# fegemo/palette-and-histo-gan

Measured on AMD Instinct MI355X. Metric: train images/sec (64x64x4 sprites), higher is better.
Workload: dtype bf16

## Files before the change

### include/p2pgan.h

```cpp
#ifndef P2PGAN_H
#define P2PGAN_H

#ifdef __cplusplus
extern "C" {
#endif

typedef enum { P2P_F32 = 0, P2P_BF16 = 1 } p2p_dtype;
typedef enum { P2P_OP_G = 0, P2P_OP_P = 1, P2P_OP_W = 2 } p2p_convop;
typedef enum { P2P_ACT_NONE = 0, P2P_ACT_LEAKY = 1, P2P_ACT_RELU = 2 } p2p_act;

typedef struct {
    void* ptr;
    long long img_stride;
    int row_stride;
    int ld;
} p2p_tensor;

typedef struct {
    const void* ptr;
    int kind;
    int nslabs;
    long long slab_stride;
    int ld;
    int coff;
} p2p_gsrc;

const char* p2p_last_error(void);
int p2p_version(void);
int p2p_view_halo_pixels(void);


int p2p_conv_direct(int op, int stride, int dtype, int N, int LH, int LW, int Cg, int Cd,
                    const p2p_tensor* hi, const p2p_tensor* lo, const void* w, const float* bias,
                    float* dw, float* dbias, void* stream);

int p2p_igemm(int op, int dtype, int N, int LH, int LW, int Cg, int Cd,
              const p2p_tensor* hi, const p2p_tensor* lo, const void* w,
              int splitk, float* slabs, float* stat_part, void* stream);
int p2p_igemm_stat_slots(int op, int N, int LH, int LW, int ncols);

int p2p_brig_ok(int op, int dtype, int N, int LH, int LW, int Cg, int Cd);
int p2p_igemm_norm_act_ok(int op, int dtype, int N, int LH, int LW, int Cg, int Cd);
int p2p_igemm_norm_act(int op, int dtype, int N, int LH, int LW, int Cg, int Cd, const p2p_tensor* hi, const p2p_tensor* lo,
                       const void* w, const float* gamma, const float* beta, float eps, int act, float alpha,
                       const p2p_tensor* act_out, float* stats, void* stream);
int p2p_brig_stat_slots(int op, int dtype, int N, int LH, int LW, int Cg, int Cd);
int p2p_igemm_layer_stat_slots(int op, int dtype, int N, int LH, int LW, int Cg, int Cd);

int p2p_igemm_edge(int op, int stride, int dtype, int N, int LH, int LW, int cin_pad, int ncols, int w_rows,
                   const p2p_tensor* in, const p2p_tensor* out, const void* w, const float* bias,
                   int act, float alpha, void* stream);

int p2p_conv_strip_ok(int op, int dtype, int N, int LH, int LW, int Cg, int Cd);
int p2p_conv_strip_stat_slots(int op, int dtype, int N, int LH, int LW, int Cg, int Cd);
int p2p_conv_strip(int op, int dtype, int N, int LH, int LW, int Cg, int Cd,
                   const p2p_tensor* hi, const p2p_tensor* lo, const void* w, float* stat_part, void* stream);

int p2p_conv_fewout_ok(int op, int stride, int dtype, int N, int LH, int LW, int cin_pad, int ncols);
int p2p_conv_fewout(int op, int stride, int dtype, int N, int LH, int LW, int cin_pad, int ncols, int w_rows,
                    const p2p_tensor* in, const p2p_tensor* out, const void* w, const float* bias,
                    int act, float alpha, void* stream);

int p2p_conv_fewin_ok(int op, int stride, int dtype, int N, int LH, int LW, int cin_pad, int ncols);
int p2p_conv_fewin(int op, int stride, int dtype, int N, int LH, int LW, int cin_pad, int ncols, int w_rows,
                   const p2p_tensor* in, const p2p_tensor* out, const void* w, const float* bias,
                   int act, float alpha, void* stream);

int p2p_conv_fewin_actbwd(int op, int stride, int dtype, int N, int LH, int LW, int cin_pad, int ncols, int w_rows,
                          const p2p_tensor* in, const p2p_tensor* out, const void* w, const p2p_tensor* gate, float alpha,
                          void* stream);

long long p2p_wgemm_workspace_bytes(int N, int LH, int LW, int Cg, int Cd, int msplit);
int p2p_wgemm(int dtype, int N, int LH, int LW, int Cg, int Cd,
              const p2p_tensor* hi, const p2p_tensor* lo, float* dw,
              int msplit, void* workspace, void* stream);

int p2p_wgemm_edge(int dtype, int stride, int N, int LH, int LW, int Cg, int Cd,
                   const p2p_tensor* hi, const p2p_tensor* lo, float* dw,
                   int msplit, void* workspace, void* stream);

int p2p_wgrad_small_blocks(int dtype, int stride, int N, int LH, int LW, int Cg, int Cd, int hi_ld, int lo_ld);
int p2p_wgrad_small(int dtype, int stride, int N, int LH, int LW, int Cg, int Cd,
                    const p2p_tensor* hi, const p2p_tensor* lo, float* dw, void* workspace, void* stream);

long long p2p_view_colsum_workspace_bytes(int dtype, int N, int H, int W, int C, const p2p_tensor* v);
int p2p_view_colsum(int dtype, int N, int H, int W, int C, const p2p_tensor* v, float* out, float* workspace, void* stream);



#define P2P_IGEMM_FAM_R03 1
#define P2P_IGEMM_FAM_GEN 2
#define P2P_IGEMM_FAM_PIPE_G 3
#define P2P_IGEMM_FAM_PIPE_P 4
#define P2P_IGEMM_TILE_128x128 0
#define P2P_IGEMM_TILE_256x128 1
#define P2P_IGEMM_TILE_128x64 2
#define P2P_IGEMM_TILE_256x64 3
#define P2P_IGEMM_TILE_128x32 4
#define P2P_IGEMM_TILE_256x32 5
#define P2P_IGEMM_ROUTE(family, tile, kgroups, stages, w_major) \
    ((family) | ((tile) << 3) | (((kgroups) - 1) << 6) | (((stages) - 2) << 7) | ((w_major) << 9))
#define P2P_IGEMM_ROUTE_BRIG 0
#define P2P_IGEMM_ARMS(X) \
    X(1, 0, 1, 2) X(1, 0, 1, 3) X(1, 1, 1, 2) X(1, 1, 1, 3) X(1, 2, 1, 2) X(1, 2, 1, 3) \
    X(1, 3, 1, 2) X(1, 3, 1, 3) X(1, 4, 1, 2) X(1, 4, 1, 3) X(1, 5, 1, 2) X(1, 5, 1, 3) \
    X(2, 0, 1, 2) X(2, 0, 1, 3) X(2, 1, 1, 2) X(2, 1, 1, 3) X(2, 2, 1, 2) X(2, 2, 1, 3) \
    X(2, 3, 1, 2) X(2, 3, 1, 3) X(2, 4, 1, 2) X(2, 4, 1, 3) X(2, 5, 1, 2) X(2, 5, 1, 3) \
    X(3, 1, 1, 3) X(3, 0, 2, 4) X(3, 0, 1, 2) X(4, 1, 1, 3) X(4, 0, 2, 4) X(4, 0, 1, 2)
int p2p_igemm_route(int op, int dtype, int N, int LH, int LW, int Cg, int Cd, const p2p_tensor* hi, const p2p_tensor* lo,
                    int splitk, int with_stats);
int p2p_igemm_edge_route(int op, int stride, int dtype, int N, int LH, int LW, int cin_pad, int ncols, int w_rows,
                         const p2p_tensor* in, const p2p_tensor* out, int with_bias, int act);

#define P2P_BRIG_ROUTE(op_p, cbw, stagger, fused) (1 | ((op_p) << 1) | (((cbw) - 1) << 2) | ((stagger) << 3) | ((fused) << 4))
#define P2P_BRIG_ROUTE_NONE 0
#define P2P_BRIG_ARMS(X) \
    X(0, 1, 0, 0) X(0, 1, 0, 1) X(0, 1, 1, 0) X(0, 1, 1, 1) X(0, 2, 0, 0) X(0, 2, 0, 1) X(0, 2, 1, 0) X(0, 2, 1, 1) \
    X(1, 1, 0, 0) X(1, 1, 0, 1) X(1, 1, 1, 0) X(1, 1, 1, 1) X(1, 2, 0, 0) X(1, 2, 0, 1) X(1, 2, 1, 0) X(1, 2, 1, 1)
int p2p_brig_route(int op, int dtype, int N, int LH, int LW, int Cg, int Cd, int fused);

#define P2P_WGEMM_ROUTE_PIPE 0
#define P2P_WGEMM_ROUTE_128x128 1
#define P2P_WGEMM_ROUTE_64x128 2
#define P2P_WGEMM_ROUTE_32x128 3
#define P2P_WGEMM_ROUTE_64x64 4
#define P2P_WGEMM_ROUTE_32x64 5
#define P2P_WGEMM_ROUTE_64x32 6
#define P2P_WGEMM_ROUTE_32x32 7
#define P2P_WGEMM_ARMS(X) X(0) X(1) X(2) X(3) X(4) X(5) X(6) X(7)
int p2p_wgemm_route(int dtype, int stride, int N, int LH, int LW, int Cg, int Cd, const p2p_tensor* hi, const p2p_tensor* lo,
                    int msplit);

#define P2P_WS_TILE_1x1 0
#define P2P_WS_TILE_1x2 1
#define P2P_WS_TILE_1x4 2
#define P2P_WS_TILE_2x1 3
#define P2P_WS_TILE_2x2 4
#define P2P_WS_ROUTE(stride, tile, waves, pack, swizzle) \
    (((stride) - 1) | ((tile) << 1) | (((waves) >> 4) << 4) | ((pack) << 5) | ((swizzle) << 7))
#define P2P_WS_ARMS(X) \
    X(1, 0, 8, 0, 0) X(1, 0, 8, 0, 1) X(1, 0, 16, 0, 0) X(1, 0, 16, 0, 1) X(1, 1, 8, 0, 0) X(1, 1, 8, 0, 1) X(1, 1, 16, 0, 0) X(1, 1, 16, 0, 1) \
    X(1, 2, 8, 0, 0) X(1, 2, 8, 0, 1) X(1, 2, 16, 0, 0) X(1, 2, 16, 0, 1) X(1, 3, 8, 0, 0) X(1, 3, 8, 0, 1) X(1, 3, 16, 0, 0) X(1, 3, 16, 0, 1) \
    X(1, 4, 8, 0, 0) X(1, 4, 8, 0, 1) X(1, 4, 16, 0, 0) X(1, 4, 16, 0, 1) \
    X(2, 0, 8, 0, 0) X(2, 0, 8, 0, 1) X(2, 0, 16, 0, 0) X(2, 0, 16, 0, 1) X(2, 1, 8, 0, 0) X(2, 1, 8, 0, 1) X(2, 1, 16, 0, 0) X(2, 1, 16, 0, 1) \
    X(2, 2, 8, 0, 0) X(2, 2, 8, 0, 1) X(2, 2, 16, 0, 0) X(2, 2, 16, 0, 1) X(2, 3, 8, 0, 0) X(2, 3, 8, 0, 1) X(2, 3, 16, 0, 0) X(2, 3, 16, 0, 1) \
    X(2, 4, 8, 0, 0) X(2, 4, 8, 0, 1) X(2, 4, 16, 0, 0) X(2, 4, 16, 0, 1) \
    X(1, 1, 8, 1, 0) X(2, 1, 8, 1, 0) X(1, 3, 8, 2, 0)
int p2p_wgrad_small_route(int dtype, int stride, int N, int LH, int LW, int Cg, int Cd, int hi_ld, int lo_ld);

#define P2P_NORM_FORM_SCALAR 0
#define P2P_NORM_FORM_SMALL 1
#define P2P_NORM_FORM_REG 2
#define P2P_NORM_FORM_VEC0 3
#define P2P_NORM_FORM_VEC12 4
#define P2P_NORM_FORM_VEC3 5
#define P2P_NORM_ROUTE(form, ppl, slabs, lg_cg) ((form) | ((ppl) << 3) | ((slabs) << 7) | ((lg_cg) << 8))
#define P2P_NORM_ROUTE_ARM(code) ((code) & 0xff)
#define P2P_NORM_FWD_ARMS(X) \
    X(0, 0, 0) X(1, 1, 0) X(1, 1, 1) X(1, 2, 0) X(1, 2, 1) X(1, 4, 0) X(1, 4, 1) \
    X(2, 1, 0) X(2, 1, 1) X(2, 2, 0) X(2, 2, 1) X(2, 4, 0) X(2, 4, 1) X(2, 8, 0) X(2, 8, 1) X(3, 0, 0) X(4, 0, 0) X(5, 0, 0)
#define P2P_NORM_BWD_ARMS(X) \
    X(0, 0, 0) X(1, 1, 0) X(1, 1, 1) X(1, 2, 0) X(1, 2, 1) X(1, 4, 0) X(1, 4, 1) \
    X(2, 1, 0) X(2, 1, 1) X(2, 2, 0) X(2, 2, 1) X(2, 4, 0) X(2, 4, 1) X(2, 8, 0) X(2, 8, 1) X(3, 0, 0) X(4, 0, 0)
int p2p_norm_act_fwd_route(int dtype, int N, int H, int W, int C, const void* raw, int raw_kind, int nslabs,
                           long long slab_stride, const float* gamma, const float* beta, const p2p_tensor* out,
                           void* raw_out, float* stats, float* ws, long long ws_bytes, int nsplit,
                           const p2p_tensor* tail, int tail_ch);
int p2p_norm_act_bwd_route(int dtype, int N, int H, int W, int C, const void* raw, const float* stats, const float* gamma,
                           const float* beta, const p2p_gsrc* g1, const p2p_gsrc* g2, const p2p_tensor* draw,
                           float* dgamma_part, float* dbeta_part, float* ws, long long ws_bytes, int nsplit);


int p2p_norm_act_fwd(int dtype, int N, int H, int W, int C,
                     const void* raw, int raw_kind, int nslabs, long long slab_stride,
                     const float* gamma, const float* beta, float eps, int act, float alpha,
                     const unsigned char* mask, const p2p_tensor* out, void* raw_out, float* stats,
                     float* ws, long long ws_bytes, int nsplit, void* stream);
int p2p_norm_act_fwd_tail(int dtype, int N, int H, int W, int C,
                          const void* raw, int raw_kind, int nslabs, long long slab_stride,
                          const float* gamma, const float* beta, float eps, int act, float alpha,
                          const unsigned char* mask, const p2p_tensor* out, void* raw_out, float* stats,
                          float* ws, long long ws_bytes, int nsplit, const p2p_tensor* tail, int tail_ch, void* stream);

int p2p_norm_act_bwd(int dtype, int N, int H, int W, int C,
                     const void* raw, const float* stats, const float* gamma, const float* beta,
                     int act, float alpha, const unsigned char* mask,
                     const p2p_gsrc* g1, const p2p_gsrc* g2,
                     const p2p_tensor* draw, float* dgamma_part, float* dbeta_part,
                     float* ws, long long ws_bytes, int nsplit, void* stream);

int p2p_norm_act_fwd_1x1(int dtype, int N, int C, const float* gamma, const float* beta, int act, float alpha,
                         const unsigned char* mask, const p2p_tensor* out, void* stream);
int p2p_norm_act_bwd_1x1(int dtype, int N, int C, const float* gamma, const float* beta, int act, float alpha,
                         const unsigned char* mask, const p2p_gsrc* g1, const p2p_gsrc* g2, float* dgamma_part,
                         float* dbeta_part, void* stream);

int p2p_act_bwd(int dtype, int N, int H, int W, int C, const p2p_tensor* act_out, const p2p_gsrc* g1,
                const p2p_gsrc* g2, float alpha, const p2p_tensor* draw, void* stream);

int p2p_colsum(const float* part, int rows, int cols, float scale, float* out, void* stream);

int p2p_colsum_batched(const float* part, const int* table, int ntasks, int max_cols, float* out, void* stream);


#define P2P_LOSS_BLOCKS 256
int p2p_loss_partials_sum(const float* partials, int K, float* out, void* stream);

int p2p_bce_logits(int dtype, int N2, int n_real, int H, int W, const p2p_tensor* logits,
                   float inv_count, const p2p_tensor* dlogits_d, const p2p_tensor* dlogits_g,
                   float* partials, void* stream);
int p2p_bce_logits_pad8(int dtype, int N2, int n_real, int H, int W, const p2p_tensor* logits,
                        float inv_count, const p2p_tensor* dlogits_d, const p2p_tensor* dlogits_g,
                        float* partials, void* stream);

int p2p_tanh_l1_fwd(int dtype, int N, int H, int W, int C, const p2p_tensor* z, const p2p_tensor* real,
                    const p2p_tensor* fake, float inv_count, float* partials, float* fake_f32, void* stream);
int p2p_tanh_l1_fwd_pair(int dtype, int N, int H, int W, const p2p_tensor* z, const p2p_tensor* real_pair,
                         const p2p_tensor* fake_pair, float inv_count, float* partials, float* fake_f32, void* stream);

int p2p_tanh_l1_bwd(int dtype, int N, int H, int W, int C, const p2p_tensor* fake, const p2p_tensor* real,
                    const p2p_gsrc* g_d, const p2p_gsrc* g_extra, float l1_scale,
                    const p2p_tensor* dz, void* stream);
int p2p_tanh_l1_bwd_pad8(int dtype, int N, int H, int W, const p2p_tensor* fake, const p2p_tensor* real,
                         const p2p_gsrc* g_d, const p2p_gsrc* g_extra, float l1_scale, const p2p_tensor* dz,
                         void* stream);


int p2p_rgbuv_hist_fwd(int dtype, int N, int H, int W, const p2p_tensor* img, float* hist, void* stream);
int p2p_rgbuv_hist_general(int dtype, int N, int H, int W, const p2p_tensor* img, int size, int method, float sigma, float* hist,
                           void* stream);

long long p2p_rgbuv_hist_fwd3_workspace_bytes(int N);
int p2p_rgbuv_hist_fwd3(int dtype, int N, int H, int W, const p2p_tensor* img, const float* points, const int* npoints, int cap,
                        float* hist, float* workspace, void* stream);
int p2p_rgbuv_points(int dtype, int N, int H, int W, const p2p_tensor* img, int cap, float* points, int* npoints, void* stream);

int p2p_hist_normalize(const float* raw, int N, float* out, void* stream);

int p2p_hellinger_fwd(const float* hist_true, const float* hist_pred, int N, float* tot_true, float* tot_pred,
                      float* sq_part, float* sq_sum, void* stream);
int p2p_hellinger_finish(const float* sq_sum, float inv_global_batch, float* loss_out, void* stream);
int p2p_rgbuv_hist_hellinger_bwd(int dtype, int N, int H, int W, const p2p_tensor* fake, const float* hist_true,
                                 const float* hist_pred, const float* tot_true, const float* tot_pred,
                                 const float* sq_sum, float coef, float* gh_ws, float* dimg, void* stream);
int p2p_rgbuv_hist_hellinger_bwd3(int dtype, int N, int H, int W, const p2p_tensor* fake, const float* hist_true,
                                  const float* hist_pred, const float* tot_true, const float* tot_pred, const float* sq_sum,
                                  float coef, float* gh_ws, float* dimg, void* stream);

int p2p_hist_normalize_bwd(const float* raw, const float* grad_out, int N, int size, float* gh, void* stream);
int p2p_rgbuv_hist_bwd(int dtype, int N, int H, int W, const p2p_tensor* img, const float* gh, float* dimg, void* stream);
int p2p_rgbuv_hist_general_bwd(int dtype, int N, int H, int W, const p2p_tensor* img, int size, int method, float sigma,
                               const float* gh, float* dimg, void* stream);

long long p2p_soft_palette_workspace_bytes(int N, int H, int W);
int p2p_soft_palette_fwd(int N, int H, int W, const float* img, const int* palette, const int* sizes, int K, float tau,
                         float* hist, float* conf, float* workspace, void* stream);
int p2p_soft_palette_bwd(int N, int H, int W, const float* img, const int* palette, const int* sizes, int K, float tau,
                         const float* gh, const float* gm, float* dimg, void* stream);
int p2p_palette_extract(int N, int H, int W, const float* img, int cap, int* palette_out, int* sizes_out, void* stream);
int p2p_palette_snap(int N, int H, int W, const float* img, const int* palette, const int* sizes, int K, int* index_out,
                     float* image_out, int* dist_out, int* counts_out, long long* stats_out, void* stream);

int p2p_palette_project_fwd(int N, int H, int W, const float* img, const int* palette, const int* sizes, int K, float tau, int hard,
                            float* out, void* stream);
int p2p_palette_project_bwd(int N, int H, int W, const float* img, const int* palette, const int* sizes, int K, float tau,
                            const float* g, float* dimg, void* stream);

long long p2p_diffaug_workspace_bytes(int N, int H, int W);
int p2p_diffaug_fwd(int N, int H, int W, const float* img, const float* color, const int* geometry, int ch, int cw,
                    int policy_bits, float fill, float* out, float* workspace, void* stream);
int p2p_diffaug_bwd(int N, int H, int W, const float* grad_out, const float* color, const int* geometry, int ch, int cw,
                    int policy_bits, float fill, float* grad_img, float* workspace, void* stream);


#define P2P_SOFTMAX_MAX_BLOCKS 8192
int p2p_softmax_cce_argmax(int dtype, int N, int H, int W, int C, const p2p_tensor* z, const p2p_tensor* target,
                           const p2p_tensor* fake_idx, float grad_scale, float inv_count, const p2p_tensor* dz,
                           float* probs_out, float* loss_part, float* loss_out, void* stream);
int p2p_softmax_bwd(int dtype, int N, int H, int W, int C, const float* probs, const float* gp, const float* gz,
                    float scale, const p2p_tensor* dz, void* stream);
int p2p_argmax_lastdim(const float* probs, long long M, int C, int* out, void* stream);

int p2p_head_softmax_ok(int dtype, int N, int H, int W, int cin_pad, int ncls);
long long p2p_head_softmax_workspace_bytes(int N, int H);
int p2p_head_softmax_cce(int dtype, int N, int H, int W, int cin_pad, int ncls, const p2p_tensor* in, const void* wt,
                         const float* bias, const p2p_tensor* target, const p2p_tensor* fake_idx, float grad_scale,
                         float inv_count, const p2p_tensor* dz, float* dbias, float* workspace, float* loss_out, void* stream);
int p2p_head_dgrad_ok(int dtype, int N, int H, int W, int ncls, int cout, int w_rows, int dz_ld, int out_ld);
int p2p_head_dgrad(int dtype, int N, int H, int W, int ncls, int cout, const p2p_tensor* dz, const void* wn, int w_rows,
                   const p2p_tensor* out, void* stream);


int p2p_adam_flat(float* p, const float* g, float* m, float* v, long long n, int t,
                  float lr, float beta1, float beta2, float eps, float gscale, void* stream);

int p2p_adam_tick(int* t_dev, float* lr_t_dev, float lr, float beta1, float beta2, void* stream);
int p2p_adam_flat_dev(float* p, const float* g, float* m, float* v, long long n, const float* lr_t_dev,
                      float beta1, float beta2, float eps, float gscale, void* stream);
int p2p_adam_flat_dev_excl(float* p, const float* g, float* m, float* v, long long n, long long ex_lo, long long ex_hi,
                           const float* lr_t_dev, float beta1, float beta2, float eps, float gscale, void* stream);
int p2p_counter_add(long long* counter_dev, long long inc, void* stream);
int p2p_grad_accumulate(float* dst, const float* src, long long n, int first, void* stream);

int p2p_weight_prep(int dtype, const float* w, int Cg, int Cd, void* wn, void* wt, void* stream);

int p2p_weight_prep_pad(int dtype, const float* w, int Cg, int Cd, void* wn, int wn_rows, int wn_cols,
                        void* wt, int wt_rows, int wt_cols, void* stream);

typedef struct p2p_prep_task {
    const float* w;
    void* wn;
    void* wt;
    int Cg, Cd, wn_rows, wn_cols, wt_rows, wt_cols, tiles_g, tiles_d;
    long long first_block;
} p2p_prep_task;
long long p2p_weight_prep_task_blocks(int Cg, int Cd, int wn_rows, int wn_cols, int wt_rows, int wt_cols,
                                      int have_wn, int have_wt, int* tiles_g, int* tiles_d);
int p2p_weight_prep_batched(int dtype, const p2p_prep_task* tasks_dev, int ntasks, long long total_blocks, void* stream);
int p2p_adam_prep_batched(int dtype, long long n_elems, const p2p_prep_task* tasks_dev, int ntasks, long long total_blocks,
                          float* params, const float* grads, float* m, float* v, const float* lr_t_dev, float beta1, float beta2,
                          float eps, void* stream);


int p2p_pack_input(int dtype, int N, int H, int W, int C, const void* src, int src_is_int,
                   const p2p_tensor* dst, void* stream);
int p2p_pack_input_multi(int dtype, int N, int H, int W, int C, const void* src, int src_is_int,
                         const p2p_tensor* dsts, int ndst, void* stream);
int p2p_pack_pair(int dtype, int N, int H, int W, const float* source, const float* target,
                  const p2p_tensor* v_src, const p2p_tensor* v_c6, const p2p_tensor* v_dreal, const p2p_tensor* v_dfake,
                  void* stream);
int p2p_pack_pair_idx(int dtype, int N, int H, int W, const int* source, const int* target,
                      const p2p_tensor* v_src, const p2p_tensor* v_c6, const p2p_tensor* v_dreal, const p2p_tensor* v_dfake,
                      void* stream);
int p2p_finish_losses(const float* slots, int aux_slot, int l1_slot, float lambda_l1, float lambda_aux, float* out,
                      void* stream);
int p2p_unpack(int dtype, int N, int H, int W, int C, const p2p_tensor* src, float* dst, void* stream);

int p2p_dropout_mask(unsigned char* mask, long long n, long long seed, long long counter, void* stream);
int p2p_dropout_mask_dev(unsigned char* mask, long long n, long long seed, const long long* counter_dev,
                         long long salt, long long elem_offset, void* stream);


int p2p_comm_unique_id(void* id_out_128_bytes);
int p2p_comm_init(const void* id_128_bytes, int rank, int world, void** comm_out);
int p2p_comm_allreduce_sum(void* comm, float* buf, long long n, void* stream);
int p2p_comm_destroy(void* comm);

int p2p_event_create(void** ev_out);
int p2p_event_destroy(void* ev);
int p2p_event_record(void* ev, void* stream);
int p2p_stream_wait_event(void* stream, void* ev);
int p2p_arm_stop_event(void* ev);
int p2p_disarm_stop_event(int* was_pending);

#define P2P_REPLAY_MAX_ARGS 24
typedef struct {
    int fn;
    int nargs;
    unsigned ind64;
    unsigned ind32;
    unsigned long long a[P2P_REPLAY_MAX_ARGS];
} p2p_replay_call;
int p2p_replay_fn_index(const char* name);
int p2p_replay_fn_nargs(int fn);
int p2p_replay(const p2p_replay_call* calls, int n);


int p2p_png_unfilter(const unsigned char* filtered, int height, int row_bytes, int bpp, unsigned char* out);

int p2p_sprites_rgba_batch(const void* sprites, int n_sprites, int S, const int* src_idx, const int* tgt_idx, const float* aug,
                           int B, int normalise, float* source, float* target, void* stream);

int p2p_gather_rows_i32(const int* table, int n_rows, int row_ints, const int* sel, int B, int* out, void* stream);

int p2p_palette_relabel_batch(const int* src_idx, const int* tgt_idx, const int* palette, const int* perm, const int* inv,
                              int B, int n, int P, int C, int* src_out, int* tgt_out, int* pal_out, void* stream);


int p2p_inc_prep(int N, int H, int W, int C, const float* images, const int* rows, const int* cols, const int* chans, int OH,
                 int OW, double w0, double w1, int filter, const p2p_tensor* out, float* minmax, void* stream);
int p2p_inc_conv(int N, int H, int W, int Cin, int kh, int kw, int stride, int pad_top, int pad_left, int OH, int OW, int Cout,
                 const p2p_tensor* in, const float* w, const float* scale, const float* shift, const p2p_tensor* out, void* stream);
int p2p_inc_pool(int kind, int N, int H, int W, int C, const p2p_tensor* in, const p2p_tensor* out, void* stream);
int p2p_inc_gap(int N, int H, int W, int C, const p2p_tensor* in, float* out, void* stream);

#ifdef __cplusplus
}
#endif
#endif
```

### palette_and_histo_gan_amd/_lib.py

```python
import ctypes as C
import os

HERE = os.path.dirname(os.path.abspath(__file__))
LIB_PATH = os.environ.get("P2P_LIB") or os.path.join(HERE, "libp2pgan_hip.so")

F32, BF16 = 0, 1
OP_G, OP_P, OP_W = 0, 1, 2
ACT_NONE, ACT_LEAKY, ACT_RELU = 0, 1, 2


class Tensor(C.Structure):
    _fields_ = [("ptr", C.c_void_p), ("img_stride", C.c_longlong), ("row_stride", C.c_int), ("ld", C.c_int)]


class GSrc(C.Structure):
    _fields_ = [("ptr", C.c_void_p), ("kind", C.c_int), ("nslabs", C.c_int), ("slab_stride", C.c_longlong),
                ("ld", C.c_int), ("coff", C.c_int)]


_TP = C.POINTER(Tensor)
_GP = C.POINTER(GSrc)
_vp, _i, _f, _ll = C.c_void_p, C.c_int, C.c_float, C.c_longlong

SIGNATURES = {
    "p2p_conv_direct": [_i, _i, _i, _i, _i, _i, _i, _i, _TP, _TP, _vp, _vp, _vp, _vp, _vp],
    "p2p_igemm": [_i, _i, _i, _i, _i, _i, _i, _TP, _TP, _vp, _i, _vp, _vp, _vp],
    "p2p_igemm_norm_act": [_i, _i, _i, _i, _i, _i, _i, _TP, _TP, _vp, _vp, _vp, _f, _i, _f, _TP, _vp, _vp],
    "p2p_igemm_edge": [_i, _i, _i, _i, _i, _i, _i, _i, _i, _TP, _TP, _vp, _vp, _i, _f, _vp],
    "p2p_conv_strip": [_i, _i, _i, _i, _i, _i, _i, _TP, _TP, _vp, _vp, _vp],
    "p2p_conv_fewin": [_i, _i, _i, _i, _i, _i, _i, _i, _i, _TP, _TP, _vp, _vp, _i, _f, _vp],
    "p2p_conv_fewin_actbwd": [_i, _i, _i, _i, _i, _i, _i, _i, _i, _TP, _TP, _vp, _TP, _f, _vp],
    "p2p_conv_fewout": [_i, _i, _i, _i, _i, _i, _i, _i, _i, _TP, _TP, _vp, _vp, _i, _f, _vp],
    "p2p_wgemm_edge": [_i, _i, _i, _i, _i, _i, _i, _TP, _TP, _vp, _i, _vp, _vp],
    "p2p_wgrad_small": [_i, _i, _i, _i, _i, _i, _i, _TP, _TP, _vp, _vp, _vp],
    "p2p_view_colsum": [_i, _i, _i, _i, _i, _TP, _vp, _vp, _vp],
    "p2p_act_bwd": [_i, _i, _i, _i, _i, _TP, _GP, _GP, _f, _TP, _vp],
    "p2p_weight_prep_pad": [_i, _vp, _i, _i, _vp, _i, _i, _vp, _i, _i, _vp],
    "p2p_wgemm": [_i, _i, _i, _i, _i, _i, _TP, _TP, _vp, _i, _vp, _vp],
    "p2p_norm_act_fwd": [_i, _i, _i, _i, _i, _vp, _i, _i, _ll, _vp, _vp, _f, _i, _f, _vp, _TP, _vp, _vp, _vp, _ll, _i, _vp],
    "p2p_norm_act_fwd_tail": [_i, _i, _i, _i, _i, _vp, _i, _i, _ll, _vp, _vp, _f, _i, _f, _vp, _TP, _vp, _vp, _vp, _ll, _i, _TP, _i, _vp],
    "p2p_norm_act_bwd": [_i, _i, _i, _i, _i, _vp, _vp, _vp, _vp, _i, _f, _vp, _GP, _GP, _TP, _vp, _vp, _vp, _ll, _i, _vp],
    "p2p_norm_act_fwd_1x1": [_i, _i, _i, _vp, _vp, _i, _f, _vp, _TP, _vp],
    "p2p_norm_act_bwd_1x1": [_i, _i, _i, _vp, _vp, _i, _f, _vp, _GP, _GP, _vp, _vp, _vp],
    "p2p_colsum": [_vp, _i, _i, _f, _vp, _vp],
    "p2p_colsum_batched": [_vp, _vp, _i, _i, _vp, _vp],
    "p2p_bce_logits": [_i, _i, _i, _i, _i, _TP, _f, _TP, _TP, _vp, _vp],
    "p2p_bce_logits_pad8": [_i, _i, _i, _i, _i, _TP, _f, _TP, _TP, _vp, _vp],
    "p2p_loss_partials_sum": [_vp, _i, _vp, _vp],
    "p2p_tanh_l1_fwd": [_i, _i, _i, _i, _i, _TP, _TP, _TP, _f, _vp, _vp, _vp],
    "p2p_tanh_l1_fwd_pair": [_i, _i, _i, _i, _TP, _TP, _TP, _f, _vp, _vp, _vp],
    "p2p_tanh_l1_bwd": [_i, _i, _i, _i, _i, _TP, _TP, _GP, _GP, _f, _TP, _vp],
    "p2p_tanh_l1_bwd_pad8": [_i, _i, _i, _i, _TP, _TP, _GP, _GP, _f, _TP, _vp],
    "p2p_adam_flat": [_vp, _vp, _vp, _vp, _ll, _i, _f, _f, _f, _f, _f, _vp],
    "p2p_adam_tick": [_vp, _vp, _f, _f, _f, _vp],
    "p2p_adam_flat_dev": [_vp, _vp, _vp, _vp, _ll, _vp, _f, _f, _f, _f, _vp],
    "p2p_adam_flat_dev_excl": [_vp, _vp, _vp, _vp, _ll, _ll, _ll, _vp, _f, _f, _f, _f, _vp],
    "p2p_counter_add": [_vp, _ll, _vp],
    "p2p_grad_accumulate": [_vp, _vp, _ll, _i, _vp],
    "p2p_dropout_mask_dev": [_vp, _ll, _ll, _vp, _ll, _ll, _vp],
    "p2p_weight_prep": [_i, _vp, _i, _i, _vp, _vp, _vp],
    "p2p_weight_prep_batched": [_i, _vp, _i, _ll, _vp],
    "p2p_adam_prep_batched": [_i, _ll, _vp, _i, _ll, _vp, _vp, _vp, _vp, _vp, _f, _f, _f, _vp],
    "p2p_pack_input": [_i, _i, _i, _i, _i, _vp, _i, _TP, _vp],
    "p2p_pack_pair": [_i, _i, _i, _i, _vp, _vp, _TP, _TP, _TP, _TP, _vp],
    "p2p_pack_pair_idx": [_i, _i, _i, _i, _vp, _vp, _TP, _TP, _TP, _TP, _vp],
    "p2p_pack_input_multi": [_i, _i, _i, _i, _i, _vp, _i, _TP, _i, _vp],
    "p2p_finish_losses": [_vp, _i, _i, _f, _f, _vp, _vp],
    "p2p_unpack": [_i, _i, _i, _i, _i, _TP, _vp, _vp],
    "p2p_dropout_mask": [_vp, _ll, _ll, _ll, _vp],
    "p2p_rgbuv_hist_fwd": [_i, _i, _i, _i, _TP, _vp, _vp],
    "p2p_hist_normalize": [_vp, _i, _vp, _vp],
    "p2p_rgbuv_hist_general": [_i, _i, _i, _i, _TP, _i, _i, _f, _vp, _vp],
    "p2p_rgbuv_hist_fwd3": [_i, _i, _i, _i, _TP, _vp, _vp, _i, _vp, _vp, _vp],
    "p2p_rgbuv_points": [_i, _i, _i, _i, _TP, _i, _vp, _vp, _vp],
    "p2p_hellinger_fwd": [_vp, _vp, _i, _vp, _vp, _vp, _vp, _vp],
    "p2p_hellinger_finish": [_vp, _f, _vp, _vp],
    "p2p_rgbuv_hist_hellinger_bwd": [_i, _i, _i, _i, _TP, _vp, _vp, _vp, _vp, _vp, _f, _vp, _vp, _vp],
    "p2p_rgbuv_hist_hellinger_bwd3": [_i, _i, _i, _i, _TP, _vp, _vp, _vp, _vp, _vp, _f, _vp, _vp, _vp],
    "p2p_hist_normalize_bwd": [_vp, _vp, _i, _i, _vp, _vp],
    "p2p_rgbuv_hist_bwd": [_i, _i, _i, _i, _TP, _vp, _vp, _vp],
    "p2p_rgbuv_hist_general_bwd": [_i, _i, _i, _i, _TP, _i, _i, _f, _vp, _vp, _vp],
    "p2p_soft_palette_fwd": [_i, _i, _i, _vp, _vp, _vp, _i, _f, _vp, _vp, _vp, _vp],
    "p2p_soft_palette_bwd": [_i, _i, _i, _vp, _vp, _vp, _i, _f, _vp, _vp, _vp, _vp],
    "p2p_palette_extract": [_i, _i, _i, _vp, _i, _vp, _vp, _vp],
    "p2p_palette_snap": [_i, _i, _i, _vp, _vp, _vp, _i, _vp, _vp, _vp, _vp, _vp, _vp],
    "p2p_palette_project_fwd": [_i, _i, _i, _vp, _vp, _vp, _i, _f, _i, _vp, _vp],
    "p2p_palette_project_bwd": [_i, _i, _i, _vp, _vp, _vp, _i, _f, _vp, _vp, _vp],
    "p2p_diffaug_fwd": [_i, _i, _i, _vp, _vp, _vp, _i, _i, _i, _f, _vp, _vp, _vp],
    "p2p_diffaug_bwd": [_i, _i, _i, _vp, _vp, _vp, _i, _i, _i, _f, _vp, _vp, _vp],
    "p2p_softmax_cce_argmax": [_i, _i, _i, _i, _i, _TP, _TP, _TP, _f, _f, _TP, _vp, _vp, _vp, _vp],
    "p2p_softmax_bwd": [_i, _i, _i, _i, _i, _vp, _vp, _vp, _f, _TP, _vp],
    "p2p_argmax_lastdim": [_vp, _ll, _i, _vp, _vp],
    "p2p_head_dgrad": [_i, _i, _i, _i, _i, _i, _TP, _vp, _i, _TP, _vp],
    "p2p_head_softmax_cce": [_i, _i, _i, _i, _i, _i, _TP, _vp, _vp, _TP, _TP, _f, _f, _TP, _vp, _vp, _vp, _vp],
    "p2p_comm_unique_id": [_vp],
    "p2p_comm_init": [_vp, _i, _i, C.POINTER(_vp)],
    "p2p_comm_allreduce_sum": [_vp, _vp, _ll, _vp],
    "p2p_comm_destroy": [_vp],
    "p2p_event_create": [C.POINTER(_vp)],
    "p2p_event_destroy": [_vp],
    "p2p_event_record": [_vp, _vp],
    "p2p_stream_wait_event": [_vp, _vp],
    "p2p_arm_stop_event": [_vp],
    "p2p_disarm_stop_event": [C.POINTER(C.c_int)],
    "p2p_png_unfilter": [_vp, _i, _i, _i, _vp],
    "p2p_sprites_rgba_batch": [_vp, _i, _i, _vp, _vp, _vp, _i, _i, _vp, _vp, _vp],
    "p2p_gather_rows_i32": [_vp, _i, _i, _vp, _i, _vp, _vp],
    "p2p_palette_relabel_batch": [_vp, _vp, _vp, _vp, _vp, _i, _i, _i, _i, _vp, _vp, _vp, _vp],
    "p2p_inc_prep": [_i, _i, _i, _i, _vp, _vp, _vp, _vp, _i, _i, C.c_double, C.c_double, _i, _TP, _vp, _vp],
    "p2p_inc_conv": [_i, _i, _i, _i, _i, _i, _i, _i, _i, _i, _i, _i, _TP, _vp, _vp, _vp, _TP, _vp],
    "p2p_inc_pool": [_i, _i, _i, _i, _i, _TP, _TP, _vp],
    "p2p_inc_gap": [_i, _i, _i, _i, _TP, _vp, _vp],
}
SPECIAL = {"p2p_last_error": ([], C.c_char_p),
           "p2p_replay_fn_index": ([C.c_char_p], C.c_int), "p2p_replay_fn_nargs": ([_i], C.c_int),
           "p2p_replay": ([_vp, _i], C.c_int), "p2p_version": ([], C.c_int), "p2p_view_halo_pixels": ([], C.c_int),
           "p2p_igemm_stat_slots": ([_i, _i, _i, _i, _i], C.c_int),
           "p2p_brig_ok": ([_i, _i, _i, _i, _i, _i, _i], C.c_int),
           "p2p_igemm_norm_act_ok": ([_i, _i, _i, _i, _i, _i, _i], C.c_int),
           "p2p_brig_stat_slots": ([_i, _i, _i, _i, _i, _i, _i], C.c_int),
           "p2p_igemm_layer_stat_slots": ([_i, _i, _i, _i, _i, _i, _i], C.c_int),
           "p2p_conv_fewin_ok": ([_i, _i, _i, _i, _i, _i, _i, _i], C.c_int),
           "p2p_conv_strip_ok": ([_i, _i, _i, _i, _i, _i, _i], C.c_int),
           "p2p_conv_strip_stat_slots": ([_i, _i, _i, _i, _i, _i, _i], C.c_int),
           "p2p_conv_fewout_ok": ([_i, _i, _i, _i, _i, _i, _i, _i], C.c_int),
           "p2p_wgrad_small_blocks": ([_i, _i, _i, _i, _i, _i, _i, _i, _i], C.c_int),
           "p2p_igemm_route": ([_i, _i, _i, _i, _i, _i, _i, _TP, _TP, _i, _i], C.c_int),
           "p2p_igemm_edge_route": ([_i, _i, _i, _i, _i, _i, _i, _i, _i, _TP, _TP, _i, _i], C.c_int),
           "p2p_brig_route": ([_i, _i, _i, _i, _i, _i, _i, _i], C.c_int),
           "p2p_wgemm_route": ([_i, _i, _i, _i, _i, _i, _i, _TP, _TP, _i], C.c_int),
           "p2p_wgrad_small_route": ([_i, _i, _i, _i, _i, _i, _i, _i, _i], C.c_int),
           "p2p_norm_act_fwd_route": ([_i, _i, _i, _i, _i, _vp, _i, _i, _ll, _vp, _vp, _TP, _vp, _vp, _vp, _ll, _i, _TP, _i], C.c_int),
           "p2p_norm_act_bwd_route": ([_i, _i, _i, _i, _i, _vp, _vp, _vp, _vp, _GP, _GP, _TP, _vp, _vp, _vp, _ll, _i], C.c_int),
           "p2p_wgemm_workspace_bytes": ([_i, _i, _i, _i, _i, _i], C.c_longlong),
           "p2p_rgbuv_hist_fwd3_workspace_bytes": ([_i], C.c_longlong),
           "p2p_soft_palette_workspace_bytes": ([_i, _i, _i], C.c_longlong),
           "p2p_diffaug_workspace_bytes": ([_i, _i, _i], C.c_longlong),
           "p2p_head_softmax_ok": ([_i, _i, _i, _i, _i, _i], C.c_int),
           "p2p_head_dgrad_ok": ([_i, _i, _i, _i, _i, _i, _i, _i, _i], C.c_int),
           "p2p_head_softmax_workspace_bytes": ([_i, _i], C.c_longlong),
           "p2p_view_colsum_workspace_bytes": ([_i, _i, _i, _i, _i, _TP], C.c_longlong),
           "p2p_weight_prep_task_blocks": ([_i, _i, _i, _i, _i, _i, _i, _i, C.POINTER(C.c_int), C.POINTER(C.c_int)], C.c_longlong)}


class PrepTask(C.Structure):
    _fields_ = [("w", C.c_void_p), ("wn", C.c_void_p), ("wt", C.c_void_p),
                ("Cg", C.c_int), ("Cd", C.c_int), ("wn_rows", C.c_int), ("wn_cols", C.c_int),
                ("wt_rows", C.c_int), ("wt_cols", C.c_int), ("tiles_g", C.c_int), ("tiles_d", C.c_int),
                ("first_block", C.c_longlong)]

_lib = None


class P2PError(RuntimeError):
    pass


def lib():
    global _lib
    if _lib is None:
        if not os.path.exists(LIB_PATH):
            raise P2PError(f"{LIB_PATH} is missing: run `python -c 'import __graft_entry__ as g; g.build()'` "
                           "(hipcc --offload-arch=gfx950); there is no CPU fallback")
        import torch
        L = C.CDLL(LIB_PATH)
        for name, argtypes in SIGNATURES.items():
            fn = getattr(L, name)
            fn.argtypes = argtypes
            fn.restype = C.c_int
        for name, (argtypes, restype) in SPECIAL.items():
            fn = getattr(L, name)
            fn.argtypes = argtypes
            fn.restype = restype
        _lib = L
    return _lib


_fns = {}


def call(name, *args):
    fn = _fns.get(name)
    if fn is None:
        fn = _fns[name] = getattr(lib(), name)
    rc = fn(*args)
    if rc != 0:
        raise P2PError(f"{name} failed (rc={rc}): {lib().p2p_last_error().decode()}")


def exported_symbols():
    return list(SIGNATURES) + list(SPECIAL)
```

### palette_and_histo_gan_amd/csrc/conv_strip.hip

```cpp
#include "p2p_common.hpp"

struct CsArgs {
    const char* in; long long in_img; int in_row; int in_ld;
    char* out; long long out_img; int out_row; int out_ld;
    const char* w;
    float* stat_part;
    int LH, LW, lgLW;
    int TH, strips_per_img, nstrips;
    int RH, RW, PB;
    float inv_RW;
};

#define CS_MAXC 7
#define CS_THREADS 512

template <int MODE>
__global__ __launch_bounds__(CS_THREADS) void conv_strip_kernel(CsArgs a) {
    constexpr int NTAP = MODE == 1 ? 4 : 16;
    constexpr int KS = MODE == 1 ? 8 : 2;
    constexpr int CIN = KS * 16;
    constexpr int LGCPP = MODE == 1 ? 4 : 2;
    constexpr int PROW = 64 + 16;
    extern __shared__ __attribute__((aligned(16))) char smem[];
    const int tid = threadIdx.x, lane = tid & 63;
    const int wave = __builtin_amdgcn_readfirstlane(tid >> 6);
    const int h = lane >> 5, r = lane & 31;
    const int RW = a.RW, PB = a.PB;
    char* sL = smem;
    char* pL = smem + ((a.RH * RW * PB + 15) & ~15) + wave * (32 * PROW);
    const int slice = wave & 3, tpar = wave >> 2;
    const int ph = slice >> 1, pw = slice & 1;

    bf16x8 wf[NTAP][KS];
#pragma unroll
    for (int t = 0; t < NTAP; ++t) {
        int widx, row;
        if (MODE == 1) { widx = ((1 - ph) + 2 * (t >> 1)) * 4 + (1 - pw) + 2 * (t & 1); row = r; }
        else { widx = t; row = 32 * slice + r; }
        const int rows = MODE == 1 ? 32 : 128;
        const char* wp = a.w + ((long long)(widx * rows + row) * CIN) * 2;
#pragma unroll
        for (int ks = 0; ks < KS; ++ks) wf[t][ks] = *(const bf16x8*)(wp + (16 * ks + 8 * h) * 2);
    }

    const int nch = (a.RH * RW) << LGCPP;
    const int gpB = a.in_ld * 2;
    f32x4 stg[CS_MAXC];
    auto g_load = [&](int strip) {
        const int n = strip / a.strips_per_img, y0 = (strip - n * a.strips_per_img) * a.TH;
        const int oy = MODE == 1 ? y0 - 1 : 2 * y0 - 1;
        const char* base = a.in + ((long long)n * a.in_img + (long long)oy * a.in_row - 1) * gpB;
#pragma unroll
        for (int i = 0; i < CS_MAXC; ++i) {
            const int ci = tid + i * CS_THREADS;
            if (ci < nch) {
                const int px = ci >> LGCPP, cc = ci & ((1 << LGCPP) - 1);
                const int ry = (int)(((float)px + 0.5f) * a.inv_RW), rx = px - ry * RW;
                stg[i] = *(const f32x4*)(base + ((long long)ry * a.in_row + rx) * gpB + cc * 16);
            }
        }
    };
    auto l_store = [&]() {
#pragma unroll
        for (int i = 0; i < CS_MAXC; ++i) {
            const int ci = tid + i * CS_THREADS;
            if (ci < nch) *(f32x4*)(sL + (ci >> LGCPP) * PB + (ci & ((1 << LGCPP) - 1)) * 16) = stg[i];
        }
    };

    const int tiles = (a.TH * a.LW) >> 5;
    float* stL = (float*)(smem + ((a.RH * RW * PB + 15) & ~15) + 8 * (32 * PROW));
    int pend_n = -1, pend_s = 0;
    auto flush_stats = [&]() {
        if (tid < 32) {
            float s1 = 0.f, s2 = 0.f;
#pragma unroll
            for (int wv = 0; wv < 8; ++wv) { s1 += stL[(wv * 32 + tid) * 2]; s2 += stL[(wv * 32 + tid) * 2 + 1]; }
            const float cnt = (float)(4 * a.TH * a.LW);
            const float mean = s1 / cnt;
            float* dst = a.stat_part + (((long long)pend_n * a.strips_per_img + pend_s) * 32 + tid) * 2;
            dst[0] = mean;
            dst[1] = fmaxf(s2 - s1 * mean, 0.f);
        }
    };
    int strip = blockIdx.x;
    if (strip < a.nstrips) g_load(strip);
    for (; strip < a.nstrips; strip += gridDim.x) {
        __syncthreads();
        if (MODE == 1 && a.stat_part && pend_n >= 0) flush_stats();
        l_store();
        __syncthreads();
        if (strip + (int)gridDim.x < a.nstrips) g_load(strip + gridDim.x);
        const int n = strip / a.strips_per_img, sidx = strip - n * a.strips_per_img, y0 = sidx * a.TH;
        float ssum = 0.f, ssq = 0.f;
        for (int tile = tpar; tile < tiles; tile += 2) {
            const int p = tile * 32 + r;
            const int yy = p >> a.lgLW, x = p & (a.LW - 1);
            f32x16 acc;
            const float zero = p2p_valu_zero();
#pragma unroll
            for (int e = 0; e < 16; ++e) acc[e] = zero;
#pragma unroll
            for (int t = 0; t < NTAP; ++t) {
                int ry, rx;
                if (MODE == 1) {
                    const int kh = (1 - ph) + 2 * (t >> 1), kw = (1 - pw) + 2 * (t & 1);
                    ry = yy + 1 + ((ph + 1 - kh) >> 1);
                    rx = x + 1 + ((pw + 1 - kw) >> 1);
                } else { ry = 2 * yy + (t >> 2); rx = 2 * x + (t & 3); }
                const char* bp = sL + (ry * RW + rx) * PB + 16 * h;
#pragma unroll
                for (int ks = 0; ks < KS; ++ks) {
                    const bf16x8 b = *(const bf16x8*)(bp + 32 * ks);
                    acc = __builtin_amdgcn_mfma_f32_32x32x16_bf16(wf[t][ks], b, acc, 0, 0, 0);
                }
            }
#pragma unroll
            for (int g = 0; g < 4; ++g) {
                typedef __attribute__((__vector_size__(4 * sizeof(bf16_t)))) bf16_t bf16x4;
                bf16x4 q;
#pragma unroll
                for (int k = 0; k < 4; ++k) q[k] = (bf16_t)acc[4 * g + k];
                *(bf16x4*)(pL + r * PROW + (8 * g + 4 * h) * 2) = q;
            }
            asm volatile("s_waitcnt lgkmcnt(0)" ::: "memory");
            __builtin_amdgcn_wave_barrier();
            if (MODE == 1 && a.stat_part) {
                const bf16_t* col = (const bf16_t*)(pL + (16 * h) * PROW) + r;
#pragma unroll
                for (int i = 0; i < 16; ++i) {
                    const float v = (float)col[i * (PROW / 2)];
                    ssum += v;
                    ssq += v * v;
                }
            }
            const int ch = lane & 3, pq = lane >> 2;
#pragma unroll
            for (int ps = 0; ps < 32; ps += 16) {
                const int pix = ps + pq;
                const int pp = tile * 32 + pix;
                const int py = pp >> a.lgLW, px = pp & (a.LW - 1);
                const f32x4 v = *(const f32x4*)(pL + pix * PROW + ch * 16);
                long long opix;
                int c0;
                if (MODE == 1) { opix = (long long)n * a.out_img + (long long)(2 * (y0 + py) + ph) * a.out_row + (2 * px + pw); c0 = ch * 8; }
                else { opix = (long long)n * a.out_img + (long long)(y0 + py) * a.out_row + px; c0 = 32 * slice + ch * 8; }
                *(f32x4*)((bf16_t*)a.out + opix * a.out_ld + c0) = v;
            }
            __builtin_amdgcn_wave_barrier();
        }
        if (MODE == 1 && a.stat_part) {
            ssum += __shfl_xor(ssum, 32, 64);
            ssq += __shfl_xor(ssq, 32, 64);
            if (h == 0) { stL[(wave * 32 + r) * 2] = ssum; stL[(wave * 32 + r) * 2 + 1] = ssq; }
            pend_n = n; pend_s = sidx;
        }
    }
    if (MODE == 1 && a.stat_part && pend_n >= 0) {
        __syncthreads();
        flush_stats();
    }
}

struct CsPlan { int ok, TH, RH, RW, PB, blocks; size_t shm; };

static CsPlan cs_plan(int op, int dtype, int N, int LH, int LW, int Cg, int Cd) {
    CsPlan p = {0, 0, 0, 0, 0, 0, 0};
    if (dtype != P2P_BF16 || Cg != 32 || Cd != 128 || N < 1) return p;
    if (op != P2P_OP_G && op != P2P_OP_P) return p;
    if ((LW & (LW - 1)) || LW < 32 || LW > 128 || LH < 1) return p;
    const int cin = op == P2P_OP_P ? 128 : 32;
    p.PB = cin * 2 + 16;
    int TH = 0;
    for (int pass = 0; pass < 2 && !TH; ++pass)
        for (int t = 4; t >= (pass ? 1 : 2); t >>= 1) {
            if (t > LH || LH % t) continue;
            p.RH = op == P2P_OP_P ? t + 2 : 2 * t + 3;
            p.RW = op == P2P_OP_P ? LW + 2 : 2 * LW + 3;
            p.shm = (((size_t)p.RH * p.RW * p.PB + 15) & ~(size_t)15) + 8 * 32 * (size_t)(64 + 16) + 8 * 32 * 2 * sizeof(float);
            const long long nch = (long long)p.RH * p.RW * (cin / 8);
            if (nch > CS_MAXC * CS_THREADS) continue;
            if (((t * LW) >> 5) & 1) continue;
            if (p.shm <= (size_t)(pass ? 150 : 80) * 1024) { TH = t; break; }
        }
    if (!TH) return p;
    p.TH = TH;
    const long long strips = (long long)N * (LH / TH);
    if (strips > 0x7fffffffLL) return p;
    p.blocks = (int)(strips < 256 ? strips : 256);
    p.ok = 1;
    return p;
}

extern "C" int p2p_conv_strip_ok(int op, int dtype, int N, int LH, int LW, int Cg, int Cd) {
    return cs_plan(op, dtype, N, LH, LW, Cg, Cd).ok;
}

extern "C" int p2p_conv_strip_stat_slots(int op, int dtype, int N, int LH, int LW, int Cg, int Cd) {
    const CsPlan p = cs_plan(op, dtype, N, LH, LW, Cg, Cd);
    return (p.ok && op == P2P_OP_P) ? LH / p.TH : 0;
}

extern "C" int p2p_conv_strip(int op, int dtype, int N, int LH, int LW, int Cg, int Cd, const p2p_tensor* hi,
                              const p2p_tensor* lo, const void* w, float* stat_part, void* stream) {
    P2P_REQUIRE(hi && lo && hi->ptr && lo->ptr && w, "p2p_conv_strip: null pointer");
    const CsPlan p = cs_plan(op, dtype, N, LH, LW, Cg, Cd);
    P2P_REQUIRE(p.ok, "p2p_conv_strip: shape not supported (query p2p_conv_strip_ok)");
    const p2p_tensor* in = op == P2P_OP_G ? hi : lo;
    const p2p_tensor* out = op == P2P_OP_G ? lo : hi;
    const int cin = op == P2P_OP_P ? 128 : 32, cout = op == P2P_OP_P ? 32 : 128;
    P2P_REQUIRE(in->ld >= cin && in->ld % 8 == 0 && ((uintptr_t)in->ptr % 16) == 0 && ((uintptr_t)w % 16) == 0,
                "p2p_conv_strip: input view / weights must be 16-byte aligned");
    P2P_REQUIRE(out->ld >= cout && out->ld % 8 == 0 && ((uintptr_t)out->ptr % 16) == 0, "p2p_conv_strip: output view must be 16-byte aligned");
    CsArgs a;
    a.in = (const char*)in->ptr; a.in_img = in->img_stride; a.in_row = in->row_stride; a.in_ld = in->ld;
    a.out = (char*)out->ptr; a.out_img = out->img_stride; a.out_row = out->row_stride; a.out_ld = out->ld;
    a.w = (const char*)w;
    a.LH = LH; a.LW = LW;
    a.lgLW = 0;
    while ((1 << a.lgLW) < LW) ++a.lgLW;
    a.TH = p.TH; a.strips_per_img = LH / p.TH; a.nstrips = N * a.strips_per_img;
    a.RH = p.RH; a.RW = p.RW; a.PB = p.PB;
    a.inv_RW = 1.0f / (float)p.RW;
    a.stat_part = op == P2P_OP_P ? stat_part : nullptr;
    hipStream_t st = (hipStream_t)stream;
    const dim3 grid((unsigned)p.blocks);
    static bool attr_done = false;
    if (!attr_done)
        attr_done = (int)p2p_allow_lds((const void*)conv_strip_kernel<0>, 160 * 1024, "conv_strip_kernel<0>") &
                    (int)p2p_allow_lds((const void*)conv_strip_kernel<1>, 160 * 1024, "conv_strip_kernel<1>");
    if (op == P2P_OP_P) conv_strip_kernel<1><<<grid, dim3(CS_THREADS), p.shm, st>>>(a);
    else conv_strip_kernel<0><<<grid, dim3(CS_THREADS), p.shm, st>>>(a);
    return p2p_check_launch("p2p_conv_strip");
}
```

Baseline: 137,100.

## Walk consecutive strips with a rolling LDS row ring to reuse halo rows

The strip conv kernel now assigns each block a segment of consecutive strips in an image and keeps the input rows in a circular LDS ring, so each step loads only the new rows instead of the full strip plus halo. The first strip is staged in two passes, the tile loop is unrolled into at most two tiles, and sched_group_barrier hints interleave LDS reads with MFMAs. This is meant to cut redundant global loads of overlapping halo rows and improve issue overlap. The cost is added ring-index arithmetic, a narrower set of supported shapes (at most four tiles per strip), and possibly less parallelism when segments get long.

```diff
diff --git a/include/p2pgan.h b/include/p2pgan.h
--- a/include/p2pgan.h
+++ b/include/p2pgan.h
@@ -53,6 +53,7 @@
 
 int p2p_conv_strip_ok(int op, int dtype, int N, int LH, int LW, int Cg, int Cd);
 int p2p_conv_strip_stat_slots(int op, int dtype, int N, int LH, int LW, int Cg, int Cd);
+int p2p_conv_strip_walk(int op, int dtype, int N, int LH, int LW, int Cg, int Cd);
 int p2p_conv_strip(int op, int dtype, int N, int LH, int LW, int Cg, int Cd,
                    const p2p_tensor* hi, const p2p_tensor* lo, const void* w, float* stat_part, void* stream);
 
diff --git a/palette_and_histo_gan_amd/_lib.py b/palette_and_histo_gan_amd/_lib.py
--- a/palette_and_histo_gan_amd/_lib.py
+++ b/palette_and_histo_gan_amd/_lib.py
@@ -123,6 +123,7 @@
            "p2p_conv_fewin_ok": ([_i, _i, _i, _i, _i, _i, _i, _i], C.c_int),
            "p2p_conv_strip_ok": ([_i, _i, _i, _i, _i, _i, _i], C.c_int),
            "p2p_conv_strip_stat_slots": ([_i, _i, _i, _i, _i, _i, _i], C.c_int),
+           "p2p_conv_strip_walk": ([_i, _i, _i, _i, _i, _i, _i], C.c_int),
            "p2p_conv_fewout_ok": ([_i, _i, _i, _i, _i, _i, _i, _i], C.c_int),
            "p2p_wgrad_small_blocks": ([_i, _i, _i, _i, _i, _i, _i, _i, _i], C.c_int),
            "p2p_igemm_route": ([_i, _i, _i, _i, _i, _i, _i, _TP, _TP, _i, _i], C.c_int),
diff --git a/palette_and_histo_gan_amd/csrc/conv_strip.hip b/palette_and_histo_gan_amd/csrc/conv_strip.hip
--- a/palette_and_histo_gan_amd/csrc/conv_strip.hip
+++ b/palette_and_histo_gan_amd/csrc/conv_strip.hip
@@ -6,12 +6,16 @@
     const char* w;
     float* stat_part;
     int LH, LW, lgLW;
-    int TH, strips_per_img, nstrips;
+    int TH, strips_per_img;
+    int segs, seg_len, units;
     int RH, RW, PB;
     float inv_RW;
 };
 
 #define CS_MAXC 7
+#define CS_NEWC 5
+#define CS_BDEPTH 6
+static_assert(CS_MAXC <= 2 * CS_NEWC, "a first strip is staged in two passes");
 #define CS_THREADS 512
 
 template <int MODE>
@@ -27,7 +31,8 @@
     const int h = lane >> 5, r = lane & 31;
     const int RW = a.RW, PB = a.PB;
     char* sL = smem;
-    char* pL = smem + ((a.RH * RW * PB + 15) & ~15) + wave * (32 * PROW);
+    const int ringB = (a.RH * RW * PB + 15) & ~15;
+    char* pL = smem + ringB + wave * (32 * PROW);
     const int slice = wave & 3, tpar = wave >> 2;
     const int ph = slice >> 1, pw = slice & 1;
 
@@ -43,17 +48,20 @@
         for (int ks = 0; ks < KS; ++ks) wf[t][ks] = *(const bf16x8*)(wp + (16 * ks + 8 * h) * 2);
     }
 
-    const int nch = (a.RH * RW) << LGCPP;
+    const int NEWR = MODE == 1 ? a.TH : 2 * a.TH;
+    const int RR = a.RH, rowB = RW * PB;
+    const int nch_first = (a.RH * RW) << LGCPP, nch_new = (NEWR * RW) << LGCPP;
     const int gpB = a.in_ld * 2;
-    f32x4 stg[CS_MAXC];
-    auto g_load = [&](int strip) {
-        const int n = strip / a.strips_per_img, y0 = (strip - n * a.strips_per_img) * a.TH;
-        const int oy = MODE == 1 ? y0 - 1 : 2 * y0 - 1;
-        const char* base = a.in + ((long long)n * a.in_img + (long long)oy * a.in_row - 1) * gpB;
-#pragma unroll
-        for (int i = 0; i < CS_MAXC; ++i) {
-            const int ci = tid + i * CS_THREADS;
-            if (ci < nch) {
+    auto opaque_tid = [&]() { int t = tid; asm volatile("" : "+v"(t)); return t; };
+    f32x4 stg[CS_NEWC];
+    int st_nch = 0, st_slot = 0, st_c0 = 0;
+    auto g_load = [&](int n, int row0) {
+        const char* base = a.in + ((long long)n * a.in_img + (long long)row0 * a.in_row - 1) * gpB;
+        const int tv = opaque_tid();
+#pragma unroll
+        for (int i = 0; i < CS_NEWC; ++i) {
+            const int ci = st_c0 + tv + i * CS_THREADS;
+            if (ci < st_nch) {
                 const int px = ci >> LGCPP, cc = ci & ((1 << LGCPP) - 1);
                 const int ry = (int)(((float)px + 0.5f) * a.inv_RW), rx = px - ry * RW;
                 stg[i] = *(const f32x4*)(base + ((long long)ry * a.in_row + rx) * gpB + cc * 16);
@@ -61,15 +69,22 @@
         }
     };
     auto l_store = [&]() {
-#pragma unroll
-        for (int i = 0; i < CS_MAXC; ++i) {
-            const int ci = tid + i * CS_THREADS;
-            if (ci < nch) *(f32x4*)(sL + (ci >> LGCPP) * PB + (ci & ((1 << LGCPP) - 1)) * 16) = stg[i];
+        const int tv = opaque_tid();
+#pragma unroll
+        for (int i = 0; i < CS_NEWC; ++i) {
+            const int ci = st_c0 + tv + i * CS_THREADS;
+            if (ci < st_nch) {
+                const int px = ci >> LGCPP, cc = ci & ((1 << LGCPP) - 1);
+                const int ry = (int)(((float)px + 0.5f) * a.inv_RW), rx = px - ry * RW;
+                int slot = st_slot + ry;
+                if (slot >= RR) slot -= RR;
+                *(f32x4*)(sL + slot * rowB + rx * PB + cc * 16) = stg[i];
+            }
         }
     };
 
     const int tiles = (a.TH * a.LW) >> 5;
-    float* stL = (float*)(smem + ((a.RH * RW * PB + 15) & ~15) + 8 * (32 * PROW));
+    float* stL = (float*)(smem + ringB + 8 * (32 * PROW));
     int pend_n = -1, pend_s = 0;
     auto flush_stats = [&]() {
         if (tid < 32) {
@@ -83,19 +98,45 @@
             dst[1] = fmaxf(s2 - s1 * mean, 0.f);
         }
     };
-    int strip = blockIdx.x;
-    if (strip < a.nstrips) g_load(strip);
-    for (; strip < a.nstrips; strip += gridDim.x) {
-        __syncthreads();
-        if (MODE == 1 && a.stat_part && pend_n >= 0) flush_stats();
+    auto first_row = [&](int sidx) { return MODE == 1 ? sidx * a.TH - 1 : 2 * sidx * a.TH - 1; };
+
+    int unit = blockIdx.x, pos = 0, base = 0;
+    int n = unit / a.segs, sidx = (unit - n * a.segs) * a.seg_len;
+    st_nch = nch_first; st_slot = 0;
+    g_load(n, first_row(sidx));
+    l_store();
+    if (nch_first > CS_NEWC * CS_THREADS) {
+        st_c0 = CS_NEWC * CS_THREADS;
+        g_load(n, first_row(sidx));
         l_store();
-        __syncthreads();
-        if (strip + (int)gridDim.x < a.nstrips) g_load(strip + gridDim.x);
-        const int n = strip / a.strips_per_img, sidx = strip - n * a.strips_per_img, y0 = sidx * a.TH;
+    }
+    __builtin_amdgcn_s_waitcnt(0x0f70);
+    __syncthreads();
+    for (;;) {
+        int nunit = unit, nk = pos + 1, nn = n, nsidx = sidx + 1, nbase = 0;
+        if (nk == a.seg_len) {
+            nunit = unit + gridDim.x; nk = 0;
+            nn = nunit / a.segs; nsidx = (nunit - nn * a.segs) * a.seg_len;
+        }
+        const bool more = nunit < a.units;
+        if (more) {
+            int row0 = first_row(nsidx);
+            st_slot = 0; st_nch = nch_first;
+            if (nk) {
+                nbase = base + NEWR;
+                if (nbase >= RR) nbase -= RR;
+                st_slot = nbase + a.RH - NEWR;
+                if (st_slot >= RR) st_slot -= RR;
+                st_nch = nch_new;
+                row0 += a.RH - NEWR;
+            }
+            st_c0 = 0;
+            g_load(nn, row0);
+        }
+        const int y0 = sidx * a.TH;
         float ssum = 0.f, ssq = 0.f;
-        for (int tile = tpar; tile < tiles; tile += 2) {
-            const int p = tile * 32 + r;
-            const int yy = p >> a.lgLW, x = p & (a.LW - 1);
+        auto do_tile = [&](int tile) __attribute__((always_inline)) {
+            const int yy = (tile * 32) >> a.lgLW, x = ((tile * 32) & (a.LW - 1)) + r;
             f32x16 acc;
             const float zero = p2p_valu_zero();
 #pragma unroll
@@ -108,13 +149,22 @@
                     ry = yy + 1 + ((ph + 1 - kh) >> 1);
                     rx = x + 1 + ((pw + 1 - kw) >> 1);
                 } else { ry = 2 * yy + (t >> 2); rx = 2 * x + (t & 3); }
-                const char* bp = sL + (ry * RW + rx) * PB + 16 * h;
+                int slot = base + ry;
+                if (slot >= RR) slot -= RR;
+                const char* bp = sL + slot * rowB + rx * PB + 16 * h;
 #pragma unroll
                 for (int ks = 0; ks < KS; ++ks) {
                     const bf16x8 b = *(const bf16x8*)(bp + 32 * ks);
                     acc = __builtin_amdgcn_mfma_f32_32x32x16_bf16(wf[t][ks], b, acc, 0, 0, 0);
                 }
             }
+            __builtin_amdgcn_sched_group_barrier(0x100, CS_BDEPTH, 0);
+#pragma unroll
+            for (int i = 0; i < NTAP * KS - CS_BDEPTH; ++i) {
+                __builtin_amdgcn_sched_group_barrier(0x008, 1, 0);
+                __builtin_amdgcn_sched_group_barrier(0x100, 1, 0);
+            }
+            __builtin_amdgcn_sched_group_barrier(0x008, CS_BDEPTH, 0);
 #pragma unroll
             for (int g = 0; g < 4; ++g) {
                 typedef __attribute__((__vector_size__(4 * sizeof(bf16_t)))) bf16_t bf16x4;
@@ -148,24 +198,37 @@
                 *(f32x4*)((bf16_t*)a.out + opix * a.out_ld + c0) = v;
             }
             __builtin_amdgcn_wave_barrier();
-        }
+        };
+        do_tile(tpar);
+        if (tiles > 2) do_tile(tpar + 2);
         if (MODE == 1 && a.stat_part) {
             ssum += __shfl_xor(ssum, 32, 64);
             ssq += __shfl_xor(ssq, 32, 64);
             if (h == 0) { stL[(wave * 32 + r) * 2] = ssum; stL[(wave * 32 + r) * 2 + 1] = ssq; }
             pend_n = n; pend_s = sidx;
         }
+        if (!more) break;
+        __syncthreads();
+        if (MODE == 1 && a.stat_part) flush_stats();
+        l_store();
+        if (nk == 0 && nch_first > CS_NEWC * CS_THREADS) {
+            st_c0 = CS_NEWC * CS_THREADS;
+            g_load(nn, first_row(nsidx));
+            l_store();
+        }
+        __syncthreads();
+        unit = nunit; pos = nk; n = nn; sidx = nsidx; base = nbase;
     }
-    if (MODE == 1 && a.stat_part && pend_n >= 0) {
+    if (MODE == 1 && a.stat_part) {
         __syncthreads();
         flush_stats();
     }
 }
 
-struct CsPlan { int ok, TH, RH, RW, PB, blocks; size_t shm; };
+struct CsPlan { int ok, TH, RH, RW, PB, segs, seg_len, units, blocks; size_t shm; };
 
 static CsPlan cs_plan(int op, int dtype, int N, int LH, int LW, int Cg, int Cd) {
-    CsPlan p = {0, 0, 0, 0, 0, 0, 0};
+    CsPlan p = {};
     if (dtype != P2P_BF16 || Cg != 32 || Cd != 128 || N < 1) return p;
     if (op != P2P_OP_G && op != P2P_OP_P) return p;
     if ((LW & (LW - 1)) || LW < 32 || LW > 128 || LH < 1) return p;
@@ -180,14 +243,22 @@
             p.shm = (((size_t)p.RH * p.RW * p.PB + 15) & ~(size_t)15) + 8 * 32 * (size_t)(64 + 16) + 8 * 32 * 2 * sizeof(float);
             const long long nch = (long long)p.RH * p.RW * (cin / 8);
             if (nch > CS_MAXC * CS_THREADS) continue;
-            if (((t * LW) >> 5) & 1) continue;
+            if ((((t * LW) >> 5) & 1) || ((t * LW) >> 5) > 4) continue;
             if (p.shm <= (size_t)(pass ? 150 : 80) * 1024) { TH = t; break; }
         }
     if (!TH) return p;
     p.TH = TH;
-    const long long strips = (long long)N * (LH / TH);
+    const int spi = LH / TH;
+    const long long strips = (long long)N * spi;
     if (strips > 0x7fffffffLL) return p;
     p.blocks = (int)(strips < 256 ? strips : 256);
+    p.segs = spi;
+    for (int s = 1; s < spi; s <<= 1)
+        if (spi % s == 0 && (long long)N * s >= p.blocks) { p.segs = s; break; }
+    p.seg_len = spi / p.segs;
+    p.units = N * p.segs;
+    const int newr = op == P2P_OP_P ? TH : 2 * TH;
+    if ((long long)newr * p.RW * (cin / 8) > CS_NEWC * CS_THREADS) return p;
     p.ok = 1;
     return p;
 }
@@ -199,6 +270,11 @@
 extern "C" int p2p_conv_strip_stat_slots(int op, int dtype, int N, int LH, int LW, int Cg, int Cd) {
     const CsPlan p = cs_plan(op, dtype, N, LH, LW, Cg, Cd);
     return (p.ok && op == P2P_OP_P) ? LH / p.TH : 0;
+}
+
+extern "C" int p2p_conv_strip_walk(int op, int dtype, int N, int LH, int LW, int Cg, int Cd) {
+    const CsPlan p = cs_plan(op, dtype, N, LH, LW, Cg, Cd);
+    return p.ok ? p.seg_len : 0;
 }
 
 extern "C" int p2p_conv_strip(int op, int dtype, int N, int LH, int LW, int Cg, int Cd, const p2p_tensor* hi,
@@ -219,7 +295,8 @@
     a.LH = LH; a.LW = LW;
     a.lgLW = 0;
     while ((1 << a.lgLW) < LW) ++a.lgLW;
-    a.TH = p.TH; a.strips_per_img = LH / p.TH; a.nstrips = N * a.strips_per_img;
+    a.TH = p.TH; a.strips_per_img = LH / p.TH;
+    a.segs = p.segs; a.seg_len = p.seg_len; a.units = p.units;
     a.RH = p.RH; a.RW = p.RW; a.PB = p.PB;
     a.inv_RW = 1.0f / (float)p.RW;
     a.stat_part = op == P2P_OP_P ? stat_part : nullptr;
```

New measurement: 137,900, median of 6. Within noise of the previous version (+0.6%).
